# flydog-sdr/FlyDog_SDR_GPS

Measured on AMD Instinct MI355X. Metric: IQ Msamples/s ingested (waterfall + GPS acq); value = GPS acq, BASELINE configs[1], higher is better.
Workload: dtype f32

## Files before the change

### flydog_sdr_gps_amd/csrc/kg_acq.hip

```cpp
#include "kg_common.h"
#include "kg_fft.h"
#include "kg_acq_tables.h"

#include <math.h>
#include <stdlib.h>
#include <vector>

#define SUB      4096
#define NTAPS    31
#define DECIM    4


enum { SRC_BITS = 0, SRC_IQ16 = 1, SRC_CHIPS = 2 };

__constant__ float c_hb_even[16] = {
    -0.010233f,  0.010668f, -0.016324f,  0.024377f, -0.036482f,  0.056990f, -0.101993f,
     0.316926f,  0.316926f, -0.101993f,  0.056990f, -0.036482f,  0.024377f, -0.016324f,
     0.010668f, -0.010233f,
};
#define HB_CENTRE 0.500009f

KG_DEV float bipolar(int bit) { return bit ? -1.0f : 1.0f; }

template <int SRC>
KG_DEV cf acq_source(const void *__restrict__ src, int i, int nvalid, int nchips, int boc)
{
    if (i >= nvalid) return cf{0.f, 0.f};
    if constexpr (SRC == SRC_BITS) {
        const uint8_t *p = (const uint8_t *) src;
        const int bit = (p[i >> 3] >> (i & 7)) & 1;
        const int ph = i & 3;
        const int ls = ph < 2, lc = (ph == 0) | (ph == 3);
        return cf{bipolar(bit ^ ls), bipolar(bit ^ lc)};
    } else if constexpr (SRC == SRC_IQ16) {
        const short2 v = ((const short2 *) src)[i];
        const float a = (float) v.x, b = (float) v.y;
        switch (i & 3) {
        case 0:  return cf{a, b};
        case 1:  return cf{b, -a};
        case 2:  return cf{-a, -b};
        default: return cf{-b, a};
        }
    } else {
        const uint8_t *p = (const uint8_t *) src;
        const int chip = p[(i >> 4) % nchips];
        const int b11 = boc ? ((i & 15) >= 8) : 0;
        return cf{bipolar(chip ^ b11), 0.f};
    }
}

KG_DEV cf hb_tap(const float2 *x)
{
    cf acc = kg_scale(kg_ld(&x[0]), c_hb_even[0]);
#pragma unroll
    for (int j = 1; j < 16; j++) acc = acc + kg_scale(kg_ld(&x[2 * j]), c_hb_even[j]);
    acc = acc + kg_scale(kg_ld(&x[(NTAPS - 1) / 2]), HB_CENTRE);
    return acc;
}

#define FE_TILE 256
#define FE_NY1  (2 * FE_TILE + NTAPS - 2)
#define FE_NX   (2 * FE_NY1 + NTAPS - 2)

template <int SRC>
__global__ __launch_bounds__(256) void acq_frontend_kernel(const uint8_t *__restrict__ src,
                                                          size_t src_stride, int nvalid, int nchips, int boc,
                                                          float2 *__restrict__ td, int fft_len)
{
    __shared__ float2 xs[FE_NX + 1];
    __shared__ float2 y1[FE_NY1 + 1];
    const int tid = threadIdx.x;
    const int o0 = blockIdx.x * FE_TILE;
    const void *s = src + (size_t) blockIdx.y * src_stride;
    for (int u = tid; u < FE_NX; u += 256) kg_st(&xs[u], acq_source<SRC>(s, 4 * o0 + u, nvalid, nchips, boc));
    __syncthreads();
    for (int u = tid; u < FE_NY1; u += 256) kg_st(&y1[u], hb_tap(&xs[2 * u]));
    __syncthreads();
    kg_st(&td[(size_t) blockIdx.y * fft_len + o0 + tid], hb_tap(&y1[2 * tid]));
}

#define STAMP(i)                                                                      \
    do {                                                                              \
        if (STAMPS) {                                                                 \
            __builtin_amdgcn_sched_barrier(0);                                        \
            if (threadIdx.x == 0 && blockIdx.x == 0 && blockIdx.y == 0)               \
                stamps[i] = __builtin_amdgcn_s_memrealtime();                         \
            __builtin_amdgcn_sched_barrier(0);                                        \
        }                                                                             \
    } while (0)

template <bool STAMPS>
__global__ __launch_bounds__(256) void acq_fft_sub_kernel(const float2 *__restrict__ td,
                                                         float2 *__restrict__ scratch,
                                                         const float2 *__restrict__ tab4096, int P,
                                                         unsigned long long *__restrict__ stamps)
{
    extern __shared__ __attribute__((aligned(16))) float2 smem[];
    const int t = threadIdx.x, g = blockIdx.x;
    const float2 *in = td + (size_t) blockIdx.y * P * SUB;
    float2 *out = scratch + ((size_t) blockIdx.y * P + g) * SUB;
    STAMP(0);
    cf x[16], y[16];
#pragma unroll
    for (int j = 0; j < 16; j++) x[j] = kg_ld(&in[P * (t + 256 * j) + g]);
    kg_tw4096 tw;
    kg_tw4096_load(tw, tab4096, t);
    if (STAMPS) { asm volatile("s_waitcnt vmcnt(0)" ::: "memory"); }
    STAMP(1);
    kg_subfft4096<-1>(x, y, smem, smem + SUB, tw, t);
    STAMP(2);
#pragma unroll
    for (int m = 0; m < 16; m++) kg_st(&out[t + 256 * m], y[m]);
    if (STAMPS) { asm volatile("s_waitcnt vmcnt(0)" ::: "memory"); }
    STAMP(3);
}

template <int P>
__global__ __launch_bounds__(256) void acq_fft_combine_kernel(const float2 *__restrict__ scratch,
                                                             float2 *__restrict__ planes,
                                                             float2 *__restrict__ planes_b,
                                                             size_t planes_stride,
                                                             const float2 *__restrict__ tabN,
                                                             int halo)
{
    static_assert(P == 4 || P == 16, "N = 16384 or 65536");
    const int k = blockIdx.x * 256 + threadIdx.x;
    const float2 *f = scratch + (size_t) blockIdx.y * (P * SUB);
    cf v[P];
    v[0] = kg_ld(&f[k]);
#pragma unroll
    for (int g = 1; g < P; g++) v[g] = kg_cmulc(kg_ld(&f[g * SUB + k]), kg_ld(&tabN[g * k]));
    cf fq[P];
    if constexpr (P == 4) {
        kg_radix4<-1>(v[0], v[1], v[2], v[3]);
#pragma unroll
        for (int q = 0; q < 4; q++) fq[q] = v[q];
    } else {
        kg_radix16<-1>(v, fq);
    }
    if (planes) {
        const int row = 2 * (256 + 2 * halo), plane = 8 * row;
        float2 *o = planes + (size_t) blockIdx.y * planes_stride + (size_t) (k & (P - 1)) * plane;
#pragma unroll
        for (int q = 0; q < P; q++) {
            const int k1 = k / P + (SUB / P) * q;
            const int tt = k1 & 255, j = k1 >> 8;
            kg_st(&o[(j >> 1) * row + 2 * (tt + halo) + (j & 1)], fq[q]);
            if (tt < halo) {
                const int jj = (j - 1) & 15;
                kg_st(&o[(jj >> 1) * row + 2 * (tt + 256 + halo) + (jj & 1)], fq[q]);
            }
            if (tt >= 256 - halo) {
                const int jj = (j + 1) & 15;
                kg_st(&o[(jj >> 1) * row + 2 * (tt - 256 + halo) + (jj & 1)], fq[q]);
            }
        }
    }
    if (planes_b) {
        const int row = 2 * (512 + 2 * halo), plane = 4 * row;
        float2 *o = planes_b + (size_t) blockIdx.y * planes_stride + (size_t) (k & (P - 1)) * plane;
#pragma unroll
        for (int q = 0; q < P; q++) {
            const int k1 = k / P + (SUB / P) * q;
            const int ii = k1 & 511, j = k1 >> 9;
            kg_st(&o[(j >> 1) * row + 2 * (ii + halo) + (j & 1)], fq[q]);
            if (ii < halo) {
                const int jj = (j - 1) & 7;
                kg_st(&o[(jj >> 1) * row + 2 * (ii + 512 + halo) + (jj & 1)], fq[q]);
            }
            if (ii >= 512 - halo) {
                const int jj = (j + 1) & 7;
                kg_st(&o[(jj >> 1) * row + 2 * (ii - 512 + halo) + (jj & 1)], fq[q]);
            }
        }
    }
}

struct acq_red { float p; int i; float s; int pad; };

#define ACQ_CLAIM_STRIDE 32
#define ACQ_LDS_BYTES (2 * SUB * sizeof(float2) + 16)

struct __attribute__((aligned(16))) acq_part { float p; int i; float s; int pad; };

struct acq_pair_desc {
    int data_off;
    int code_off;
    int limit;
    int out;
};

struct acq_cell_desc { int data_off, code_off, dop, limit, out; };

struct acq_walk {
    int npairs;
    int ndop, dop_lo;
};

template <int P, bool STAMPS = false>
__global__ __launch_bounds__(256, 2) void acq_correlate_kernel(
    const float2 *__restrict__ data,
    const float2 *__restrict__ code,
    const float2 *__restrict__ tab4096, const float2 *__restrict__ tabN,
    const float2 *__restrict__ comb,
    const acq_pair_desc *__restrict__ pairs,
    int *__restrict__ claim,
    acq_walk walk,
    int halo,
    acq_part *__restrict__ parts,
    unsigned long long *__restrict__ stamps = nullptr)
{
    static_assert(P == 4 || P == 16, "N = 16384 or 65536");
    constexpr int LOGP = P == 4 ? 2 : 4;
    extern __shared__ __attribute__((aligned(16))) float2 smem[];
    float2 *tileA = smem, *tileB = smem + SUB;
    typedef __attribute__((address_space(3))) volatile int acq_lds_int;
    acq_lds_int *claim_slot = (acq_lds_int *) (smem + 2 * SUB);
    const int t = threadIdx.x;
    unsigned long long *st = (STAMPS && t == 0 && blockIdx.x == 8) ? stamps : nullptr;
    if (STAMPS && st) { st[0] = __builtin_amdgcn_s_memtime(); st[1] = __builtin_amdgcn_s_memrealtime(); }
    unsigned long long *wgt = (STAMPS && t == 0) ? stamps + 512 + 4 * blockIdx.x : nullptr;
    int wg_cells = 0;
    if (STAMPS && wgt) {
        wgt[0] = __builtin_amdgcn_s_memrealtime();
        wgt[2] = (unsigned long long) __builtin_amdgcn_s_getreg((20 << 0) | (0 << 6) | (31 << 11));
    }

    kg_tw4096 tw;
// ... 555 lines not shown
            const acq_part a1 = w[1], b1 = w[3];
            auto merge = [](acq_part &x, const acq_part &o) {
                const bool take = (o.p > x.p) | ((o.p == x.p) & (o.i < x.i));
                x.p = take ? o.p : x.p; x.i = take ? o.i : x.i;
                x.s += o.s;
            };
            merge(a, a1); merge(b, b1); merge(a, b);
            const float ave = a.s / (float) pd.limit;
            c.snr = a.p / ave;
            c.max_pwr = a.p; c.tot_pwr = a.s; c.idx = a.i;
            cells[(size_t) pd.out + di] = c;
        } else {
            c = cells[(size_t) pd.out + di];
        }
        if (c.snr > bs) { bs = c.snr; bd = di; bidx = c.idx; }
    }
#pragma unroll
    for (int off = 32; off >= 1; off >>= 1) {
        const float os = __shfl_xor(bs, off);
        const int od = __shfl_xor(bd, off), oi = __shfl_xor(bidx, off);
        if (os > bs || (os == bs && od < bd)) { bs = os; bd = od; bidx = oi; }
    }
    if (lane == 0) {
        kg_acq_result r;
        r.valid = bs > 0.f ? 1 : 0;
        r.snr = r.valid ? bs : 0.f;
        r.dop = r.valid ? dop_lo + bd : 0;
        r.idx = r.valid ? bidx : 0;
        out[p] = r;
    }
}

struct kg_acq {
    kg_ctx *ctx;
    int max_sats, dop_lo, dop_hi, ndop, max_blocks;
    int nsamples;
    int fft_len;
    int P;
    size_t in_stride;
    int halo;
    size_t code_len;
    const float2 *d_tabN;
    kg_dbuf<float2> own_tabN;
    kg_dbuf<float2> d_comb;
    kg_dbuf<float2> d_quart;
    kg_dbuf<float2> d_comb8;
    int grid8;
    kg_dbuf<float2> d_code;
    kg_dbuf<float2> d_data;
    kg_dbuf<float2> d_data_b;
    std::vector<char> code_layout;
    kg_dbuf<float2> d_td;
    kg_dbuf<float2> d_td_code;
    kg_dbuf<float2> d_fsub;
    kg_dbuf<float2> d_fsub_code;
    kg_dbuf<uint8_t> d_in;
    kg_hbuf<uint8_t> h_pin[4];
    hipEvent_t ev_pin[4];
    int pin_next;
    kg_hbuf<uint8_t> h_batch; size_t batch_cap; hipEvent_t ev_batch;
    hipStream_t cstream; hipEvent_t ev_in_free; bool in_free_set;
    kg_dbuf<uint8_t> d_chips;
    kg_dbuf<kg_acq_cell> d_cells;
    kg_dbuf<acq_part> d_parts;
    kg_dbuf<kg_acq_result> d_results;
    kg_dbuf<int> d_claim;
    std::vector<int> limits, code_set;
    std::vector<int> last_sats;
    const acq_pair_desc *d_pairs1, *d_pairs4;
    unsigned long pairs_seq;
    int last_first, last_nblocks, last_nsats, np1, np4, table_nblocks;
    hipStream_t fstream;
    bool own_fstream;
    std::vector<hipEvent_t> ev_ready, ev_done;
    std::vector<int> ready_of, done_of;
    int grid1;
};

static inline __host__ __device__ size_t plane_pos(int k1, int halo_col, int H, int layout)
{
    if (layout == 0) {
        const int t = k1 & 255, j = k1 >> 8, row = 2 * (256 + 2 * H);
        return (size_t) (j >> 1) * row + 2 * (t + halo_col + H) + (j & 1);
    }
    const int t = k1 & 511, j = k1 >> 9, row = 2 * (512 + 2 * H);
    return (size_t) (j >> 1) * row + 2 * (t + halo_col + H) + (j & 1);
}
static inline size_t spec_len(int P, int H) { return (size_t) P * 8 * 2 * (256 + 2 * H); }
static inline __host__ __device__ size_t plane_len(int H, int layout) { return layout == 0 ? (size_t) 8 * 2 * (256 + 2 * H) : (size_t) 4 * 2 * (512 + 2 * H); }

__global__ void acq_code_overrun_kernel(float2 *__restrict__ dst, int layout_dst, const float2 *__restrict__ src, int layout_src, int P, int H)
{
    const int t = blockIdx.x * blockDim.x + threadIdx.x;
    if (t >= P * H) return;
    const int k2 = t % P, k1 = t / P;
    const float2 v = src ? src[(size_t) k2 * plane_len(H, layout_src) + plane_pos(k1, 0, H, layout_src)] : make_float2(0.f, 0.f);
    const int T = layout_dst == 0 ? 256 : 512, J = SUB / T;
    dst[(size_t) k2 * plane_len(H, layout_dst) + plane_pos(k1 + T * (J - 1), T, H, layout_dst)] = v;
}

static void to_planes(const float *nat, std::vector<float2> &pl, int P, int H, int layout)
{
    const size_t plane = plane_len(H, layout);
    const int T = layout == 0 ? 256 : 512, J = SUB / T;
    pl.assign(spec_len(P, H), make_float2(0.f, 0.f));
    for (int k = 0; k < P * SUB; k++) {
        const float2 v = make_float2(nat[2 * k], nat[2 * k + 1]);
        const int k1 = k / P, t = k1 & (T - 1), j = k1 / T;
        float2 *p = pl.data() + (size_t) (k % P) * plane;
        p[plane_pos(k1, 0, H, layout)] = v;
        if (t < H) p[plane_pos(t + T * ((j - 1) & (J - 1)), T, H, layout)] = v;
        if (t >= T - H) p[plane_pos(t + T * ((j + 1) & (J - 1)), -T, H, layout)] = v;
    }
}
static void from_planes(const std::vector<float2> &pl, float *nat, int P, int H, int layout)
{
    const size_t plane = plane_len(H, layout);
    for (int k = 0; k < P * SUB; k++) {
        const float2 v = pl[(size_t) (k % P) * plane + plane_pos(k / P, 0, H, layout)];
        nat[2 * k] = v.x; nat[2 * k + 1] = v.y;
    }
}

static float2 unit_root(long k, long n)
{
    float2 r;
    kg_unit_root_f(k, n, &r.x, &r.y);
    return r;
}

template <int SRC>
static int launch_frontend(kg_acq *a, hipStream_t st, const uint8_t *d_src, size_t stride, int nbatch,
                           int nvalid, int nchips, int boc, float2 *d_td, float2 *d_scratch,
                           float2 *d_planes, float2 *d_planes_b, size_t planes_stride, int halo)
{
    kg_ctx *c = a->ctx;
    hipLaunchKernelGGL(acq_frontend_kernel<SRC>, dim3(a->fft_len / FE_TILE, nbatch), dim3(256), 0,
                       st, d_src, stride, nvalid, nchips, boc, d_td, a->fft_len);
    KG_HIP(hipGetLastError());
    hipLaunchKernelGGL(acq_fft_sub_kernel<false>, dim3(a->P, nbatch), dim3(256), 2 * SUB * sizeof(float2),
                       st, (const float2 *) d_td, d_scratch, (const float2 *) c->d_tab4096, a->P,
                       (unsigned long long *) nullptr);
    KG_HIP(hipGetLastError());
    if (a->P == 4)
        hipLaunchKernelGGL(acq_fft_combine_kernel<4>, dim3(SUB / 256, nbatch), dim3(256), 0, st,
                           (const float2 *) d_scratch, d_planes, d_planes_b, planes_stride,
                           (const float2 *) a->d_tabN, halo);
    else
        hipLaunchKernelGGL(acq_fft_combine_kernel<16>, dim3(SUB / 256, nbatch), dim3(256), 0, st,
                           (const float2 *) d_scratch, d_planes, d_planes_b, planes_stride,
                           (const float2 *) a->d_tabN, halo);
    KG_HIP(hipGetLastError());
    return KG_OK;
}

static int acq_init(kg_acq *a)
{
    kg_ctx *ctx = a->ctx;
    const int max_sats = a->max_sats, max_blocks = a->max_blocks, N = a->fft_len, P = a->P;
    {
        const int m = (a->dop_hi > -a->dop_lo ? a->dop_hi : -a->dop_lo);
        a->halo = (m + P - 1) / P + 2;
        a->code_len = spec_len(P, a->halo);
    }
    a->limits.assign(max_sats, 0); a->code_set.assign(max_sats, 0); a->code_layout.assign(max_sats, 0);
    a->last_first = a->last_nblocks = a->last_nsats = a->np1 = a->np4 = a->table_nblocks = 0;
    a->d_pairs1 = a->d_pairs4 = nullptr; a->pairs_seq = 0;
    a->in_stride = (size_t) a->nsamples * 4;
    const size_t spec = sizeof(float2) * N;
    if (N == 16384) a->d_tabN = ctx->d_tab16384;
    else {
        std::vector<float2> h(N);
        for (int k = 0; k < N; k++) h[k] = unit_root(k, N);
        KG_TRY(a->own_tabN.alloc(N, "kg_acq_create: twiddle table"));
        a->d_tabN = a->own_tabN;
        KG_HIP(hipMemcpy(a->own_tabN, h.data(), spec, hipMemcpyHostToDevice));
    }
    {
        std::vector<float2> comb(P * KG_ACQ_ROWK + (P == 16 ? 4 * 256 : 0)), quart(P * 4);
        static_assert(sizeof(float2) == 2 * sizeof(float), "float2 = (re, im)");
        kg_acq_row_consts(P, &comb[0].x);
        if (P == 16) kg_acq_mid_factors(N, &comb[P * KG_ACQ_ROWK].x);
        for (int k2 = 0; k2 < P; k2++)
            for (int q = 0; q < 4; q++) quart[4 * k2 + q] = unit_root((long) q * k2, P);
        KG_TRY(a->d_comb.alloc(comb.size(), "kg_acq_create: row constants"));
        KG_TRY(a->d_quart.alloc(quart.size(), "kg_acq_create: quarter factors"));
        KG_HIP(hipMemcpy(a->d_comb, comb.data(), sizeof(float2) * comb.size(), hipMemcpyHostToDevice));
        KG_HIP(hipMemcpy(a->d_quart, quart.data(), sizeof(float2) * quart.size(), hipMemcpyHostToDevice));
        std::vector<float2> comb8(P * 4);
        for (int k2 = 0; k2 < P; k2++)
            for (int k = 0; k < 4; k++) comb8[4 * k2 + k] = unit_root((long) (k + 1) * k2, N / 512);
        KG_TRY(a->d_comb8.alloc(comb8.size(), "kg_acq_create: combine constants"));
        KG_HIP(hipMemcpy(a->d_comb8, comb8.data(), sizeof(float2) * comb8.size(), hipMemcpyHostToDevice));
    }
    KG_TRY(a->d_code.alloc(a->code_len * max_sats, "kg_acq_create: code spectra"));
    KG_TRY(a->d_data.alloc((size_t) N * max_blocks, "kg_acq_create: data spectra"));
    KG_TRY(a->d_td.alloc((size_t) N * max_blocks, "kg_acq_create: decimated samples"));
    KG_TRY(a->d_td_code.alloc(N, "kg_acq_create: decimated samples"));
    KG_TRY(a->d_fsub.alloc((size_t) N * max_blocks, "kg_acq_create: sub-transforms"));
    KG_TRY(a->d_fsub_code.alloc(N, "kg_acq_create: sub-transforms"));
    KG_TRY(a->d_in.alloc(a->in_stride * max_blocks, "kg_acq_create: input staging"));
    for (int k = 0; k < 4; k++) {
        KG_TRY(a->h_pin[k].alloc(a->in_stride, "kg_acq_create: pinned input slots"));
        KG_HIP(hipEventCreateWithFlags(&a->ev_pin[k], hipEventDisableTiming));
    }
    KG_HIP(hipEventCreateWithFlags(&a->ev_batch, hipEventDisableTiming));
    KG_HIP(hipEventCreateWithFlags(&a->ev_in_free, hipEventDisableTiming));
    KG_TRY(kg_stream_get(ctx->device, &a->cstream));
    KG_TRY(a->d_chips.alloc(8192, "kg_acq_create: chips"));
    KG_TRY(a->d_cells.alloc((size_t) max_blocks * max_sats * a->ndop, "kg_acq_create: cells"));
    KG_TRY(a->d_parts.alloc(4 * (size_t) max_blocks * max_sats * a->ndop, "kg_acq_create: wave records"));
    KG_TRY(a->d_results.alloc((size_t) max_blocks * max_sats, "kg_acq_create: results"));
    KG_TRY(a->d_claim.alloc(16 * ACQ_CLAIM_STRIDE, "kg_acq_create: claim counters"));
    KG_HIP(hipMemset(a->d_claim, 0, sizeof(int) * 16 * ACQ_CLAIM_STRIDE));
    {
        const char *e = kg_tuning_env("KIWIGPU_ACQ_FRONT_STREAM");
        if (e && e[0] == '1') {
            KG_TRY(kg_stream_get(ctx->device, &a->fstream));
            a->own_fstream = true;
        }
    }
    a->ready_of.assign(max_blocks, -1); a->done_of.assign(max_blocks, -1);
    a->ev_ready.reserve(max_blocks); a->ev_done.reserve(max_blocks);
    for (int b = 0; b < max_blocks; b++) {
        hipEvent_t e1, e2;
        KG_HIP(hipEventCreateWithFlags(&e1, hipEventDisableTiming));
        a->ev_ready.push_back(e1);
        KG_HIP(hipEventCreateWithFlags(&e2, hipEventDisableTiming));
        a->ev_done.push_back(e2);
    }
    KG_HIP(hipMemset(a->d_data, 0, spec * max_blocks));
    KG_HIP(hipFuncSetAttribute((const void *) acq_fft_sub_kernel<false>,
                               hipFuncAttributeMaxDynamicSharedMemorySize, 2 * SUB * sizeof(float2)));
    KG_HIP(hipFuncSetAttribute((const void *) acq_fft_sub_kernel<true>,
                               hipFuncAttributeMaxDynamicSharedMemorySize, 2 * SUB * sizeof(float2)));
    int occ1 = 0;
#define ACQ_SETUP(PP)                                                                                          \
    KG_HIP(hipFuncSetAttribute((const void *) acq_correlate_kernel<PP>,                                       \
                               hipFuncAttributeMaxDynamicSharedMemorySize, ACQ_LDS_BYTES));                   \
    KG_HIP(hipOccupancyMaxActiveBlocksPerMultiprocessor(&occ1, acq_correlate_kernel<PP>, 256,                 \
                                                        ACQ_LDS_BYTES));
    if (P == 4) { ACQ_SETUP(4) } else { ACQ_SETUP(16) }
#undef ACQ_SETUP
    if (occ1 < 1) occ1 = 1;
    if (const char *e = kg_tuning_env("KIWIGPU_ACQ_WGS_PER_CU")) {
        const int v = atoi(e);
        if (v >= 1 && v < occ1) occ1 = v;
    }
    a->grid1 = (ctx->num_cus * occ1) & ~7;
    if (P == 4)
        KG_HIP(hipFuncSetAttribute((const void *) acq_correlate8_kernel<4>,
                                   hipFuncAttributeMaxDynamicSharedMemorySize, ACQ8_LDS_BYTES));
    else
        KG_HIP(hipFuncSetAttribute((const void *) acq_correlate8_kernel<16>,
                                   hipFuncAttributeMaxDynamicSharedMemorySize, ACQ8_LDS_BYTES));
    a->grid8 = ctx->num_cus & ~7;
    if (a->grid8 < 8) a->grid8 = 8;
    if (a->grid1 < 8) a->grid1 = 8;
    return KG_OK;
}

extern "C" {

int kg_acq_create_shape(kg_ctx *ctx, int max_sats, int dop_lo, int dop_hi, int max_blocks, int nsamples,
                        int fft_len, kg_acq **out)
{
    int rc = kg_ctx_use(ctx);
    if (rc) return rc;
    KG_REQUIRE(out != nullptr, KG_ERR_INVALID, "kg_acq_create: out is null");
    *out = nullptr;
    KG_REQUIRE(max_sats >= 1 && max_sats <= 4096, KG_ERR_INVALID, "kg_acq_create: max_sats %d", max_sats);
    KG_REQUIRE(dop_lo <= dop_hi && dop_lo >= -1000 && dop_hi <= 1000, KG_ERR_INVALID,
               "kg_acq_create: Doppler range %d..%d (supported: within -1000..1000)", dop_lo, dop_hi);
    KG_REQUIRE(max_blocks >= 1 && max_blocks <= 65535, KG_ERR_INVALID, "kg_acq_create: max_blocks %d",
               max_blocks);
    KG_REQUIRE(fft_len == 16384 || fft_len == 65536, KG_ERR_INVALID,
               "kg_acq_create: fft_len %d (supported: 16384, 65536)", fft_len);
    KG_REQUIRE(nsamples >= 8 && nsamples <= DECIM * fft_len && nsamples % 8 == 0, KG_ERR_INVALID,
               "kg_acq_create: nsamples %d (a multiple of 8, at most %d)", nsamples, DECIM * fft_len);
    KG_REQUIRE((size_t) max_blocks * fft_len < ((size_t) 1 << 31), KG_ERR_INVALID,
               "kg_acq_create: max_blocks %d x fft_len %d exceeds the 2^31-element offset range", max_blocks, fft_len);
    kg_acq *a = new (std::nothrow) kg_acq();
    KG_REQUIRE(a != nullptr, KG_ERR_NOMEM, "kg_acq_create: alloc");
    a->ctx = ctx; a->max_sats = max_sats; a->dop_lo = dop_lo; a->dop_hi = dop_hi;
    a->ndop = dop_hi - dop_lo + 1; a->max_blocks = max_blocks;
    a->nsamples = nsamples; a->fft_len = fft_len; a->P = fft_len / SUB;
    a->fstream = ctx->stream;
    rc = acq_init(a);
// ... 44 lines not shown
        from_planes(pl, nat.data(), a->P, 0, 0);
        to_planes(nat.data(), plb, a->P, 0, 1);
        memcpy(all.data() + (size_t) b * a->fft_len, plb.data(), sizeof(float2) * a->fft_len);
    }
    KG_REQUIRE(hipMemcpy(d, all.data(), sizeof(float2) * n, hipMemcpyHostToDevice) == hipSuccess, KG_ERR_HIP,
               "ensure_data_b: upload of layout B failed");
    a->d_data_b.p = d.p; d.p = nullptr;
    return KG_OK;
}

static int set_limit(kg_acq *a, int sat, int limit)
{
    KG_REQUIRE(sat >= 0 && sat < a->max_sats, KG_ERR_INVALID, "sat %d out of range (0..%d)", sat,
               a->max_sats - 1);
    KG_REQUIRE(limit >= 1 && limit <= 4 * SUB, KG_ERR_INVALID, "limit %d out of range (1..%d)", limit,
               4 * SUB);
    const int layout = limit > SUB ? 1 : 0;
    if (layout) {
        int rc = ensure_data_b(a);
        if (rc) return rc;
    }
    a->limits[sat] = limit;
    a->code_layout[sat] = layout;
    a->code_set[sat] = 1;
    a->last_sats.clear();
    return KG_OK;
}

static int acq_patch_overrun(kg_acq *a, int sat)
{
    if (sat < 0 || sat >= a->max_sats || !a->code_set[sat]) return KG_OK;
    const bool have_next = sat + 1 < a->max_sats && a->code_set[sat + 1];
    const int n = a->P * a->halo;
    hipLaunchKernelGGL(acq_code_overrun_kernel, dim3((n + 63) / 64), dim3(64), 0, a->ctx->stream,
                       a->d_code + (size_t) sat * a->code_len, a->code_layout[sat],
                       have_next ? (const float2 *) (a->d_code + (size_t) (sat + 1) * a->code_len) : (const float2 *) nullptr,
                       have_next ? a->code_layout[sat + 1] : 0, a->P, a->halo);
    KG_HIP(hipGetLastError());
    return KG_OK;
}

int kg_acq_set_code(kg_acq *a, int sat, const uint8_t *chips, int nchips, int boc, int limit)
{
    KG_REQUIRE(a && chips, KG_ERR_INVALID, "kg_acq_set_code: null argument");
    int rc = kg_ctx_use(a->ctx);
    if (rc) return rc;
    KG_REQUIRE(nchips >= 1 && nchips <= 8192, KG_ERR_INVALID, "kg_acq_set_code: nchips %d", nchips);
    for (int i = 0; i < nchips; i++)
        KG_REQUIRE(chips[i] <= 1, KG_ERR_INVALID, "kg_acq_set_code: chips[%d] = %d is not 0/1", i, chips[i]);
    KG_TRY(set_limit(a, sat, limit));
    KG_HIP(hipMemcpyAsync(a->d_chips, chips, nchips, hipMemcpyHostToDevice, a->ctx->stream));
    float2 *d_sv = a->d_code + (size_t) sat * a->code_len;
    rc = launch_frontend<SRC_CHIPS>(a, a->ctx->stream, a->d_chips, 0, 1, DECIM * a->fft_len, nchips, boc ? 1 : 0,
                                    a->d_td_code, a->d_fsub_code, a->code_layout[sat] ? nullptr : d_sv,
                                    a->code_layout[sat] ? d_sv : nullptr, a->code_len, a->halo);
    if (rc) return rc;
    if ((rc = acq_patch_overrun(a, sat)) || (rc = acq_patch_overrun(a, sat - 1))) return rc;
    KG_HIP(hipStreamSynchronize(a->ctx->stream));
    return KG_OK;
}

int kg_acq_set_code_fft(kg_acq *a, int sat, const float *code_fft, int limit)
{
    KG_REQUIRE(a && code_fft, KG_ERR_INVALID, "kg_acq_set_code_fft: null argument");
    int rc = kg_ctx_use(a->ctx);
    if (rc) return rc;
    KG_TRY(set_limit(a, sat, limit));
    std::vector<float2> pl;
    to_planes(code_fft, pl, a->P, a->halo, a->code_layout[sat]);
    KG_HIP(hipMemcpyAsync(a->d_code + (size_t) sat * a->code_len, pl.data(), sizeof(float2) * a->code_len,
                          hipMemcpyHostToDevice, a->ctx->stream));
    if ((rc = acq_patch_overrun(a, sat)) || (rc = acq_patch_overrun(a, sat - 1))) return rc;
    KG_HIP(hipStreamSynchronize(a->ctx->stream));
    return KG_OK;
}

static int get_planes(kg_acq *a, const float2 *d, float *nat, int H, int layout)
{
    std::vector<float2> pl(spec_len(a->P, H));
    KG_HIP(hipStreamSynchronize(a->fstream));
    KG_HIP(hipMemcpyAsync(pl.data(), d, sizeof(float2) * pl.size(), hipMemcpyDeviceToHost, a->ctx->stream));
    KG_HIP(hipStreamSynchronize(a->ctx->stream));
    from_planes(pl, nat, a->P, H, layout);
    return KG_OK;
}

int kg_acq_get_code_fft(kg_acq *a, int sat, float *code_fft)
{
    KG_REQUIRE(a && code_fft, KG_ERR_INVALID, "kg_acq_get_code_fft: null argument");
    int rc = kg_ctx_use(a->ctx);
    if (rc) return rc;
    KG_REQUIRE(sat >= 0 && sat < a->max_sats, KG_ERR_INVALID, "kg_acq_get_code_fft: sat %d", sat);
    KG_REQUIRE(a->code_set[sat], KG_ERR_STATE, "kg_acq_get_code_fft: no code set for sat %d", sat);
    return get_planes(a, a->d_code + (size_t) sat * a->code_len, code_fft, a->halo, a->code_layout[sat]);
}

static int check_block(kg_acq *a, int block, const void *p, const char *who)
{
    KG_REQUIRE(a && p, KG_ERR_INVALID, "%s: null argument", who);
    KG_REQUIRE(block >= 0 && block < a->max_blocks, KG_ERR_INVALID, "%s: block %d out of range (0..%d)",
               who, block, a->max_blocks - 1);
    return kg_ctx_use(a->ctx);
}

__global__ __launch_bounds__(256) void acq_stage_copy_kernel(const uint4 *__restrict__ src, uint4 *__restrict__ dst, size_t n16)
{
    const size_t i = (size_t) blockIdx.x * 256 + threadIdx.x;
// ... 7 lines not shown
    KG_HIP(hipEventSynchronize(a->ev_pin[k]));
    memcpy(a->h_pin[k], src, bytes);
    if ((bytes & 15) == 0 && bytes >= 65536) {
        const size_t n16 = bytes / 16;
        hipLaunchKernelGGL(acq_stage_copy_kernel, dim3((unsigned) ((n16 + 255) / 256)), dim3(256), 0, a->fstream,
                           (const uint4 *) a->h_pin[k].p, (uint4 *) d_stage, n16);
        KG_HIP(hipGetLastError());
    } else {
        KG_HIP(hipMemcpyAsync(d_stage, a->h_pin[k], bytes, hipMemcpyHostToDevice, a->fstream));
    }
    KG_HIP(hipEventRecord(a->ev_pin[k], a->fstream));
    return KG_OK;
}
static int staging_consumed(kg_acq *a)
{
    KG_HIP(hipEventRecord(a->ev_in_free, a->fstream));
    a->in_free_set = true;
    return KG_OK;
}

static int wait_once(hipStream_t st, const std::vector<hipEvent_t> &ev, const std::vector<int> &of, int b, int n)
{
    for (int i = b; i < b + n; i++) {
        const int e = of[i];
        if (e < 0) continue;
        bool seen = false;
        for (int k = b; k < i && !seen; k++) seen = of[k] == e;
        if (!seen) KG_HIP(hipStreamWaitEvent(st, ev[e], 0));
    }
    return KG_OK;
}
static int front_begin(kg_acq *a, int b, int n = 1)
{
    if (!a->own_fstream) return KG_OK;
    return wait_once(a->fstream, a->ev_done, a->done_of, b, n);
}
static int front_end(kg_acq *a, int b, int n = 1)
{
    if (!a->own_fstream) return KG_OK;
    KG_HIP(hipEventRecord(a->ev_ready[b], a->fstream));
    for (int i = b; i < b + n; i++) a->ready_of[i] = b;
    return KG_OK;
}

}

template <int SRC>
static int sample_dev(kg_acq *a, int first, int nblocks, const void *d_src, size_t stride)
{
    int rc;
    KG_TRY(front_begin(a, first, nblocks));
    const size_t off = (size_t) first * a->fft_len;
    rc = launch_frontend<SRC>(a, a->fstream, (const uint8_t *) d_src, stride, nblocks, a->nsamples, 0, 0,
                              a->d_td + off, a->d_fsub + off, a->d_data + off, a->d_data_b ? a->d_data_b + off : nullptr,
                              a->fft_len, 0);
    if (rc) return rc;
    return front_end(a, first, nblocks);
}

extern "C" {

int kg_acq_sample_bits_dev(kg_acq *a, int block, const void *d_packed)
{
    int rc = check_block(a, block, d_packed, "kg_acq_sample_bits_dev");
    if (rc) return rc;
    return sample_dev<SRC_BITS>(a, block, 1, d_packed, 0);
}

int kg_acq_sample_bits(kg_acq *a, int block, const uint8_t *packed)
{
    int rc = check_block(a, block, packed, "kg_acq_sample_bits");
    if (rc) return rc;
    uint8_t *stage = a->d_in + a->in_stride * block;
    if ((rc = stage_host_block(a, stage, packed, (size_t) a->nsamples / 8))) return rc;
    KG_TRY(sample_dev<SRC_BITS>(a, block, 1, stage, 0));
    return staging_consumed(a);
}

int kg_acq_sample_iq16_dev(kg_acq *a, int block, const void *d_iq)
{
    int rc = check_block(a, block, d_iq, "kg_acq_sample_iq16_dev");
    if (rc) return rc;
    KG_REQUIRE(((uintptr_t) d_iq & 3) == 0, KG_ERR_INVALID, "kg_acq_sample_iq16_dev: pointer not 4-byte aligned");
    return sample_dev<SRC_IQ16>(a, block, 1, d_iq, 0);
}

int kg_acq_sample_iq16_batch_dev(kg_acq *a, int first, int nblocks, const void *d_iq, size_t stride_bytes)
{
    int rc = check_block(a, first, d_iq, "kg_acq_sample_iq16_batch_dev");
    if (rc) return rc;
    KG_REQUIRE(nblocks >= 1 && first + nblocks <= a->max_blocks, KG_ERR_INVALID,
               "kg_acq_sample_iq16_batch_dev: blocks %d..%d (max %d)", first, first + nblocks - 1, a->max_blocks);
    KG_REQUIRE(((uintptr_t) d_iq & 3) == 0 && (stride_bytes & 3) == 0, KG_ERR_INVALID,
               "kg_acq_sample_iq16_batch_dev: pointer/stride not 4-byte aligned");
    return sample_dev<SRC_IQ16>(a, first, nblocks, d_iq, stride_bytes);
}

int kg_acq_sample_iq16_batch(kg_acq *a, int first, int nblocks, const int16_t *iq, size_t stride_samples)
{
    int rc = check_block(a, first, iq, "kg_acq_sample_iq16_batch");
    if (rc) return rc;
    KG_REQUIRE(nblocks >= 1 && first + nblocks <= a->max_blocks, KG_ERR_INVALID,
               "kg_acq_sample_iq16_batch: blocks %d..%d (max %d)", first, first + nblocks - 1, a->max_blocks);
    KG_REQUIRE(stride_samples >= (size_t) a->nsamples, KG_ERR_INVALID, "kg_acq_sample_iq16_batch: stride %zu < %d samples",
               stride_samples, a->nsamples);
    const size_t bytes = a->in_stride * (size_t) nblocks;
    KG_HIP(hipEventSynchronize(a->ev_batch));
// ... 203 lines not shown
        if (a->P == 4) {
            KG_HIP(hipFuncSetAttribute((const void *) acq_correlate8_kernel<4, true>,
                                       hipFuncAttributeMaxDynamicSharedMemorySize, ACQ8_LDS_BYTES));
            hipLaunchKernelGGL((acq_correlate8_kernel<4, true>), dim3(a->grid8), dim3(512), ACQ8_LDS_BYTES, st,
                               (const float2 *) a->d_data_b, (const float2 *) a->d_code, (const float2 *) a->ctx->d_tab4096,
                               (const float2 *) a->d_tabN, (const float2 *) a->d_comb8, (const float2 *) a->d_quart,
                               a->d_pairs4, a->d_claim + 8 * ACQ_CLAIM_STRIDE, w, a->halo, a->d_cells, d);
        } else {
            KG_HIP(hipFuncSetAttribute((const void *) acq_correlate8_kernel<16, true>,
                                       hipFuncAttributeMaxDynamicSharedMemorySize, ACQ8_LDS_BYTES));
            hipLaunchKernelGGL((acq_correlate8_kernel<16, true>), dim3(a->grid8), dim3(512), ACQ8_LDS_BYTES, st,
                               (const float2 *) a->d_data_b, (const float2 *) a->d_code, (const float2 *) a->ctx->d_tab4096,
                               (const float2 *) a->d_tabN, (const float2 *) a->d_comb8, (const float2 *) a->d_quart,
                               a->d_pairs4, a->d_claim + 8 * ACQ_CLAIM_STRIDE, w, a->halo, a->d_cells, d);
        }
        KG_HIP(hipGetLastError());
        KG_HIP(hipMemsetAsync(a->d_claim, 0, sizeof(int) * 16 * ACQ_CLAIM_STRIDE, st));
        KG_HIP(hipStreamSynchronize(st));
        KG_HIP(hipMemcpy(stamps, d, bytes, hipMemcpyDeviceToHost));
        return KG_OK;
    }
    KG_REQUIRE(a->np1 > 0, KG_ERR_STATE, "kg_acq_debug_corr_stamps: no C/A SV in the list");
    unsigned long long *d = nullptr;
    const size_t bytes = sizeof(unsigned long long) * (512 + 4 * 1024);
    KG_REQUIRE(a->grid1 <= 1024, KG_ERR_STATE, "kg_acq_debug_corr_stamps: grid %d", a->grid1);
    kg_scope tmp(a->ctx);
    KG_TRY(tmp.alloc(&d, 512 + 4 * 1024, "kg_acq_debug_corr_stamps"));
    KG_HIP(hipMemset(d, 0, bytes));
    KG_HIP(hipMemsetAsync(a->d_claim, 0, sizeof(int) * 16 * ACQ_CLAIM_STRIDE, st));
    if (a->P == 4) {
        KG_HIP(hipFuncSetAttribute((const void *) acq_correlate_kernel<4, true>,
                                   hipFuncAttributeMaxDynamicSharedMemorySize, ACQ_LDS_BYTES));
        launch_correlate<4, true>(a, st, 0, a->d_pairs1, a->np1, d);
    } else {
        KG_HIP(hipFuncSetAttribute((const void *) acq_correlate_kernel<16, true>,
                                   hipFuncAttributeMaxDynamicSharedMemorySize, ACQ_LDS_BYTES));
        launch_correlate<16, true>(a, st, 0, a->d_pairs1, a->np1, d);
    }
    KG_HIP(hipGetLastError());
    KG_HIP(hipMemsetAsync(a->d_claim, 0, sizeof(int) * 16 * ACQ_CLAIM_STRIDE, st));
    KG_HIP(hipStreamSynchronize(st));
    KG_HIP(hipMemcpy(stamps, d, bytes, hipMemcpyDeviceToHost));
    return KG_OK;
}

int kg_acq_debug_fft_stamps(kg_acq *a, int block, unsigned long long *stamps, int n)
{
    int rc = check_block(a, block, stamps, "kg_acq_debug_fft_stamps");
    if (rc) return rc;
    KG_REQUIRE(n >= 4, KG_ERR_INVALID, "kg_acq_debug_fft_stamps: need room for 4 stamps");
    kg_ctx *c = a->ctx;
    unsigned long long *d = nullptr;
    kg_scope tmp(c);
    KG_TRY(tmp.alloc(&d, 8, "kg_acq_debug_fft_stamps"));
    KG_HIP(hipStreamSynchronize(a->fstream));
    for (int rep = 0; rep < 3; rep++) {
        hipLaunchKernelGGL(acq_fft_sub_kernel<true>, dim3(a->P, 1), dim3(256), 2 * SUB * sizeof(float2),
                           c->stream, (const float2 *) (a->d_td + (size_t) block * a->fft_len),
                           a->d_fsub + (size_t) block * a->fft_len, (const float2 *) c->d_tab4096, a->P, d);
        KG_HIP(hipGetLastError());
        KG_HIP(hipStreamSynchronize(c->stream));
    }
    KG_HIP(hipMemcpy(stamps, d, 4 * sizeof(unsigned long long), hipMemcpyDeviceToHost));
    return KG_OK;
}

}
```

Baseline: 2674.

## Fuse FFT sub-transforms and combine into one decimation-in-frequency forward kernel

Replaces the two-pass FFT (4096-point sub-FFTs on strided inputs written to scratch, then a radix-4/16 combine kernel scattering into correlation planes) with one kernel. Each block first does the radix-P butterfly plus twiddle on contiguous loads, then a 4096-point FFT, and writes plane rows directly with vectorized stores. This removes the scratch buffer round trip and one launch. It also restructures the half-band decimation front end into polyphase even/odd LDS layouts with per-thread register taps and vector output stores. The cost is more register pressure and redundant global reads in the P=16 path, since each block reloads all 16 segments.

```diff
diff --git a/flydog_sdr_gps_amd/csrc/kg_acq.hip b/flydog_sdr_gps_amd/csrc/kg_acq.hip
--- a/flydog_sdr_gps_amd/csrc/kg_acq.hip
+++ b/flydog_sdr_gps_amd/csrc/kg_acq.hip
@@ -49,34 +49,62 @@
     }
 }
 
-KG_DEV cf hb_tap(const float2 *x)
-{
-    cf acc = kg_scale(kg_ld(&x[0]), c_hb_even[0]);
-#pragma unroll
-    for (int j = 1; j < 16; j++) acc = acc + kg_scale(kg_ld(&x[2 * j]), c_hb_even[j]);
-    acc = acc + kg_scale(kg_ld(&x[(NTAPS - 1) / 2]), HB_CENTRE);
-    return acc;
+template <int K>
+KG_DEV void hb_taps(const cf (&e)[K + 15], const cf (&o)[K], cf (&y)[K])
+{
+#pragma unroll
+    for (int k = 0; k < K; k++) {
+        cf acc = kg_scale(e[k], c_hb_even[0]);
+#pragma unroll
+        for (int j = 1; j < 16; j++) acc = acc + kg_scale(e[k + j], c_hb_even[j]);
+        y[k] = acc + kg_scale(o[k], HB_CENTRE);
+    }
 }
 
 #define FE_TILE 256
 #define FE_NY1  (2 * FE_TILE + NTAPS - 2)
 #define FE_NX   (2 * FE_NY1 + NTAPS - 2)
+#define FE_XS 168
+#define FE_YS 144
 
 template <int SRC>
 __global__ __launch_bounds__(256) void acq_frontend_kernel(const uint8_t *__restrict__ src,
                                                           size_t src_stride, int nvalid, int nchips, int boc,
                                                           float2 *__restrict__ td, int fft_len)
 {
-    __shared__ float2 xs[FE_NX + 1];
-    __shared__ float2 y1[FE_NY1 + 1];
+    __shared__ float2 xe[4 * FE_XS], xo[4 * FE_XS];
+    __shared__ __attribute__((aligned(16))) float2 ye[2 * FE_YS], yo[2 * FE_YS];
     const int tid = threadIdx.x;
     const int o0 = blockIdx.x * FE_TILE;
     const void *s = src + (size_t) blockIdx.y * src_stride;
-    for (int u = tid; u < FE_NX; u += 256) kg_st(&xs[u], acq_source<SRC>(s, 4 * o0 + u, nvalid, nchips, boc));
+    for (int u = tid; u < FE_NX; u += 256) {
+        const int i = u >> 1;
+        kg_st(&((u & 1) ? xo : xe)[(i & 3) * FE_XS + (i >> 2)], acq_source<SRC>(s, 4 * o0 + u, nvalid, nchips, boc));
+    }
     __syncthreads();
-    for (int u = tid; u < FE_NY1; u += 256) kg_st(&y1[u], hb_tap(&xs[2 * u]));
+    if (tid < (FE_NY1 + 3) / 4) {
+        cf e[19], o[4], y[4];
+#pragma unroll
+        for (int m = 0; m < 19; m++) e[m] = kg_ld(&xe[(m & 3) * FE_XS + tid + (m >> 2)]);
+#pragma unroll
+        for (int k = 0; k < 4; k++) o[k] = kg_ld(&xo[((7 + k) & 3) * FE_XS + tid + ((7 + k) >> 2)]);
+        hb_taps<4>(e, o, y);
+        kg_st(&ye[tid], y[0]);
+        if (4 * tid + 1 < FE_NY1) kg_st(&yo[tid], y[1]);
+        if (4 * tid + 2 < FE_NY1) kg_st(&ye[FE_YS + tid], y[2]);
+        if (4 * tid + 3 < FE_NY1) kg_st(&yo[FE_YS + tid], y[3]);
+    }
     __syncthreads();
-    kg_st(&td[(size_t) blockIdx.y * fft_len + o0 + tid], hb_tap(&y1[2 * tid]));
+    if (tid < FE_TILE / 2) {
+        cf e[17], o[2], y[2];
+#pragma unroll
+        for (int m = 0; m < 17; m++) e[m] = kg_ld(&ye[(m & 1) * FE_YS + tid + (m >> 1)]);
+#pragma unroll
+        for (int k = 0; k < 2; k++) o[k] = kg_ld(&yo[((7 + k) & 1) * FE_YS + tid + ((7 + k) >> 1)]);
+        hb_taps<2>(e, o, y);
+        typedef float cf2 __attribute__((ext_vector_type(4)));
+        *reinterpret_cast<cf2 *>(&td[(size_t) blockIdx.y * fft_len + o0 + 2 * tid]) = cf2{y[0].x, y[0].y, y[1].x, y[1].y};
+    }
 }
 
 #define STAMP(i)                                                                      \
@@ -89,91 +117,121 @@
         }                                                                             \
     } while (0)
 
-template <bool STAMPS>
-__global__ __launch_bounds__(256) void acq_fft_sub_kernel(const float2 *__restrict__ td,
-                                                         float2 *__restrict__ scratch,
-                                                         const float2 *__restrict__ tab4096, int P,
-                                                         unsigned long long *__restrict__ stamps)
-{
+KG_DEV cf acq_radix4_out(cf x0, cf x1, cf x2, cf x3, int r)
+{
+    if (r & 1) {
+        const cf d02 = x0 - x2, d13 = x1 - x3;
+        return (r & 2) ? kg_addj(d02, d13) : kg_subj(d02, d13);
+    }
+    const cf s02 = x0 + x2, s13 = x1 + x3;
+    return (r & 2) ? s02 - s13 : s02 + s13;
+}
+
+KG_DEV void acq_store_plane(const cf (&y)[16], float2 *__restrict__ pa, float2 *__restrict__ pb, int t, int halo)
+{
+    typedef float cf2 __attribute__((ext_vector_type(4)));
+    if (pa) {
+        const int row = 2 * (256 + 2 * halo);
+#pragma unroll
+        for (int i = 0; i < 8; i++)
+            *reinterpret_cast<cf2 *>(&pa[i * row + 2 * (t + halo)]) = cf2{y[2 * i].x, y[2 * i].y, y[2 * i + 1].x, y[2 * i + 1].y};
+        if (t < halo) {
+#pragma unroll
+            for (int j = 0; j < 16; j++) {
+                const int jj = (j - 1) & 15;
+                kg_st(&pa[(jj >> 1) * row + 2 * (t + 256 + halo) + (jj & 1)], y[j]);
+            }
+        }
+        if (t >= 256 - halo) {
+#pragma unroll
+            for (int j = 0; j < 16; j++) {
+                const int jj = (j + 1) & 15;
+                kg_st(&pa[(jj >> 1) * row + 2 * (t - 256 + halo) + (jj & 1)], y[j]);
+            }
+        }
+    }
+    if (pb) {
+        const int row = 2 * (512 + 2 * halo);
+#pragma unroll
+        for (int i = 0; i < 8; i++) {
+            const int m = 4 * (i >> 1) + (i & 1);
+            *reinterpret_cast<cf2 *>(&pb[(i >> 1) * row + 2 * (t + 256 * (i & 1) + halo)]) =
+                cf2{y[m].x, y[m].y, y[m + 2].x, y[m + 2].y};
+        }
+        if (t < halo) {
+#pragma unroll
+            for (int j = 0; j < 8; j++) {
+                const int jj = (j - 1) & 7;
+                kg_st(&pb[(jj >> 1) * row + 2 * (t + 512 + halo) + (jj & 1)], y[2 * j]);
+            }
+        }
+        if (t >= 256 - halo) {
+#pragma unroll
+            for (int j = 0; j < 8; j++) {
+                const int jj = (j + 1) & 7;
+                kg_st(&pb[(jj >> 1) * row + 2 * (t - 256 + halo) + (jj & 1)], y[2 * j + 1]);
+            }
+        }
+    }
+}
+
+template <int P, bool STAMPS>
+__global__ __launch_bounds__(256) void acq_fft_forward_kernel(const float2 *__restrict__ td,
+                                                             float2 *__restrict__ planes,
+                                                             float2 *__restrict__ planes_b,
+                                                             size_t planes_stride,
+                                                             const float2 *__restrict__ tab4096,
+                                                             const float2 *__restrict__ tabN,
+                                                             int halo,
+                                                             unsigned long long *__restrict__ stamps)
+{
+    static_assert(P == 4 || P == 16, "N = 16384 or 65536");
     extern __shared__ __attribute__((aligned(16))) float2 smem[];
-    const int t = threadIdx.x, g = blockIdx.x;
-    const float2 *in = td + (size_t) blockIdx.y * P * SUB;
-    float2 *out = scratch + ((size_t) blockIdx.y * P + g) * SUB;
+    const int t = threadIdx.x, r = blockIdx.x;
+    const float2 *in = td + (size_t) blockIdx.y * (P * SUB);
     STAMP(0);
     cf x[16], y[16];
-#pragma unroll
-    for (int j = 0; j < 16; j++) x[j] = kg_ld(&in[P * (t + 256 * j) + g]);
+    if constexpr (P == 4) {
+        cf a[4][16];
+#pragma unroll
+        for (int q = 0; q < 4; q++)
+#pragma unroll
+            for (int j = 0; j < 16; j++) a[q][j] = kg_ld(&in[SUB * q + t + 256 * j]);
+#pragma unroll
+        for (int j = 0; j < 16; j++) x[j] = acq_radix4_out(a[0][j], a[1][j], a[2][j], a[3][j], r);
+    } else {
+        const cf w1 = kg_ld(&tabN[(r & 15) * (SUB * P / 16)]), w2 = kg_ld(&tabN[((2 * r) & 15) * (SUB * P / 16)]),
+                 w3 = kg_ld(&tabN[((3 * r) & 15) * (SUB * P / 16)]);
+#pragma unroll
+        for (int j = 0; j < 16; j++) {
+            cf a[16];
+#pragma unroll
+            for (int q = 0; q < 16; q++) a[q] = kg_ld(&in[SUB * q + t + 256 * j]);
+            cf u[4];
+#pragma unroll
+            for (int b = 0; b < 4; b++) u[b] = acq_radix4_out(a[b], a[4 + b], a[8 + b], a[12 + b], r & 3);
+            kg_cmul3v<true>(u[1], u[2], u[3], w1, w2, w3);
+            x[j] = (u[0] + u[2]) + (u[1] + u[3]);
+        }
+    }
+    if (r) {
+        cf w[16];
+#pragma unroll
+        for (int j = 0; j < 16; j++) w[j] = kg_ld(&tabN[r * (t + 256 * j)]);
+#pragma unroll
+        for (int j = 0; j < 16; j += 4) kg_cmul4v<true>(x[j], x[j + 1], x[j + 2], x[j + 3], w[j], w[j + 1], w[j + 2], w[j + 3]);
+    }
     kg_tw4096 tw;
     kg_tw4096_load(tw, tab4096, t);
     if (STAMPS) { asm volatile("s_waitcnt vmcnt(0)" ::: "memory"); }
     STAMP(1);
     kg_subfft4096<-1>(x, y, smem, smem + SUB, tw, t);
     STAMP(2);
-#pragma unroll
-    for (int m = 0; m < 16; m++) kg_st(&out[t + 256 * m], y[m]);
+    const size_t spec = (size_t) blockIdx.y * planes_stride;
+    acq_store_plane(y, planes ? planes + spec + (size_t) r * (8 * 2 * (256 + 2 * halo)) : nullptr,
+                    planes_b ? planes_b + spec + (size_t) r * (4 * 2 * (512 + 2 * halo)) : nullptr, t, halo);
     if (STAMPS) { asm volatile("s_waitcnt vmcnt(0)" ::: "memory"); }
     STAMP(3);
-}
-
-template <int P>
-__global__ __launch_bounds__(256) void acq_fft_combine_kernel(const float2 *__restrict__ scratch,
-                                                             float2 *__restrict__ planes,
-                                                             float2 *__restrict__ planes_b,
-                                                             size_t planes_stride,
-                                                             const float2 *__restrict__ tabN,
-                                                             int halo)
-{
-    static_assert(P == 4 || P == 16, "N = 16384 or 65536");
-    const int k = blockIdx.x * 256 + threadIdx.x;
-    const float2 *f = scratch + (size_t) blockIdx.y * (P * SUB);
-    cf v[P];
-    v[0] = kg_ld(&f[k]);
-#pragma unroll
-    for (int g = 1; g < P; g++) v[g] = kg_cmulc(kg_ld(&f[g * SUB + k]), kg_ld(&tabN[g * k]));
-    cf fq[P];
-    if constexpr (P == 4) {
-        kg_radix4<-1>(v[0], v[1], v[2], v[3]);
-#pragma unroll
-        for (int q = 0; q < 4; q++) fq[q] = v[q];
-    } else {
-        kg_radix16<-1>(v, fq);
-    }
-    if (planes) {
-        const int row = 2 * (256 + 2 * halo), plane = 8 * row;
-        float2 *o = planes + (size_t) blockIdx.y * planes_stride + (size_t) (k & (P - 1)) * plane;
-#pragma unroll
-        for (int q = 0; q < P; q++) {
-            const int k1 = k / P + (SUB / P) * q;
-            const int tt = k1 & 255, j = k1 >> 8;
-            kg_st(&o[(j >> 1) * row + 2 * (tt + halo) + (j & 1)], fq[q]);
-            if (tt < halo) {
-                const int jj = (j - 1) & 15;
-                kg_st(&o[(jj >> 1) * row + 2 * (tt + 256 + halo) + (jj & 1)], fq[q]);
-            }
-            if (tt >= 256 - halo) {
-                const int jj = (j + 1) & 15;
-                kg_st(&o[(jj >> 1) * row + 2 * (tt - 256 + halo) + (jj & 1)], fq[q]);
-            }
-        }
-    }
-    if (planes_b) {
-        const int row = 2 * (512 + 2 * halo), plane = 4 * row;
-        float2 *o = planes_b + (size_t) blockIdx.y * planes_stride + (size_t) (k & (P - 1)) * plane;
-#pragma unroll
-        for (int q = 0; q < P; q++) {
-            const int k1 = k / P + (SUB / P) * q;
-            const int ii = k1 & 511, j = k1 >> 9;
-            kg_st(&o[(j >> 1) * row + 2 * (ii + halo) + (j & 1)], fq[q]);
-            if (ii < halo) {
-                const int jj = (j - 1) & 7;
-                kg_st(&o[(jj >> 1) * row + 2 * (ii + 512 + halo) + (jj & 1)], fq[q]);
-            }
-            if (ii >= 512 - halo) {
-                const int jj = (j + 1) & 7;
-                kg_st(&o[(jj >> 1) * row + 2 * (ii - 512 + halo) + (jj & 1)], fq[q]);
-            }
-        }
-    }
 }
 
 struct acq_red { float p; int i; float s; int pad; };
@@ -835,8 +893,6 @@
     std::vector<char> code_layout;
     kg_dbuf<float2> d_td;
     kg_dbuf<float2> d_td_code;
-    kg_dbuf<float2> d_fsub;
-    kg_dbuf<float2> d_fsub_code;
     kg_dbuf<uint8_t> d_in;
     kg_hbuf<uint8_t> h_pin[4];
     hipEvent_t ev_pin[4];
@@ -914,25 +970,21 @@
 
 template <int SRC>
 static int launch_frontend(kg_acq *a, hipStream_t st, const uint8_t *d_src, size_t stride, int nbatch,
-                           int nvalid, int nchips, int boc, float2 *d_td, float2 *d_scratch,
+                           int nvalid, int nchips, int boc, float2 *d_td,
                            float2 *d_planes, float2 *d_planes_b, size_t planes_stride, int halo)
 {
     kg_ctx *c = a->ctx;
     hipLaunchKernelGGL(acq_frontend_kernel<SRC>, dim3(a->fft_len / FE_TILE, nbatch), dim3(256), 0,
                        st, d_src, stride, nvalid, nchips, boc, d_td, a->fft_len);
     KG_HIP(hipGetLastError());
-    hipLaunchKernelGGL(acq_fft_sub_kernel<false>, dim3(a->P, nbatch), dim3(256), 2 * SUB * sizeof(float2),
-                       st, (const float2 *) d_td, d_scratch, (const float2 *) c->d_tab4096, a->P,
-                       (unsigned long long *) nullptr);
-    KG_HIP(hipGetLastError());
     if (a->P == 4)
-        hipLaunchKernelGGL(acq_fft_combine_kernel<4>, dim3(SUB / 256, nbatch), dim3(256), 0, st,
-                           (const float2 *) d_scratch, d_planes, d_planes_b, planes_stride,
-                           (const float2 *) a->d_tabN, halo);
+        hipLaunchKernelGGL((acq_fft_forward_kernel<4, false>), dim3(4, nbatch), dim3(256), 2 * SUB * sizeof(float2), st,
+                           (const float2 *) d_td, d_planes, d_planes_b, planes_stride, (const float2 *) c->d_tab4096,
+                           (const float2 *) a->d_tabN, halo, (unsigned long long *) nullptr);
     else
-        hipLaunchKernelGGL(acq_fft_combine_kernel<16>, dim3(SUB / 256, nbatch), dim3(256), 0, st,
-                           (const float2 *) d_scratch, d_planes, d_planes_b, planes_stride,
-                           (const float2 *) a->d_tabN, halo);
+        hipLaunchKernelGGL((acq_fft_forward_kernel<16, false>), dim3(16, nbatch), dim3(256), 2 * SUB * sizeof(float2), st,
+                           (const float2 *) d_td, d_planes, d_planes_b, planes_stride, (const float2 *) c->d_tab4096,
+                           (const float2 *) a->d_tabN, halo, (unsigned long long *) nullptr);
     KG_HIP(hipGetLastError());
     return KG_OK;
 }
@@ -980,8 +1032,6 @@
     KG_TRY(a->d_data.alloc((size_t) N * max_blocks, "kg_acq_create: data spectra"));
     KG_TRY(a->d_td.alloc((size_t) N * max_blocks, "kg_acq_create: decimated samples"));
     KG_TRY(a->d_td_code.alloc(N, "kg_acq_create: decimated samples"));
-    KG_TRY(a->d_fsub.alloc((size_t) N * max_blocks, "kg_acq_create: sub-transforms"));
-    KG_TRY(a->d_fsub_code.alloc(N, "kg_acq_create: sub-transforms"));
     KG_TRY(a->d_in.alloc(a->in_stride * max_blocks, "kg_acq_create: input staging"));
     for (int k = 0; k < 4; k++) {
         KG_TRY(a->h_pin[k].alloc(a->in_stride, "kg_acq_create: pinned input slots"));
@@ -1013,10 +1063,12 @@
         a->ev_done.push_back(e2);
     }
     KG_HIP(hipMemset(a->d_data, 0, spec * max_blocks));
-    KG_HIP(hipFuncSetAttribute((const void *) acq_fft_sub_kernel<false>,
-                               hipFuncAttributeMaxDynamicSharedMemorySize, 2 * SUB * sizeof(float2)));
-    KG_HIP(hipFuncSetAttribute((const void *) acq_fft_sub_kernel<true>,
-                               hipFuncAttributeMaxDynamicSharedMemorySize, 2 * SUB * sizeof(float2)));
+    if (P == 4)
+        KG_HIP(hipFuncSetAttribute((const void *) acq_fft_forward_kernel<4, false>,
+                                   hipFuncAttributeMaxDynamicSharedMemorySize, 2 * SUB * sizeof(float2)));
+    else
+        KG_HIP(hipFuncSetAttribute((const void *) acq_fft_forward_kernel<16, false>,
+                                   hipFuncAttributeMaxDynamicSharedMemorySize, 2 * SUB * sizeof(float2)));
     int occ1 = 0;
 #define ACQ_SETUP(PP)                                                                                          \
     KG_HIP(hipFuncSetAttribute((const void *) acq_correlate_kernel<PP>,                                       \
@@ -1167,7 +1219,7 @@
     KG_HIP(hipMemcpyAsync(a->d_chips, chips, nchips, hipMemcpyHostToDevice, a->ctx->stream));
     float2 *d_sv = a->d_code + (size_t) sat * a->code_len;
     rc = launch_frontend<SRC_CHIPS>(a, a->ctx->stream, a->d_chips, 0, 1, DECIM * a->fft_len, nchips, boc ? 1 : 0,
-                                    a->d_td_code, a->d_fsub_code, a->code_layout[sat] ? nullptr : d_sv,
+                                    a->d_td_code, a->code_layout[sat] ? nullptr : d_sv,
                                     a->code_layout[sat] ? d_sv : nullptr, a->code_len, a->halo);
     if (rc) return rc;
     if ((rc = acq_patch_overrun(a, sat)) || (rc = acq_patch_overrun(a, sat - 1))) return rc;
@@ -1281,7 +1333,7 @@
     KG_TRY(front_begin(a, first, nblocks));
     const size_t off = (size_t) first * a->fft_len;
     rc = launch_frontend<SRC>(a, a->fstream, (const uint8_t *) d_src, stride, nblocks, a->nsamples, 0, 0,
-                              a->d_td + off, a->d_fsub + off, a->d_data + off, a->d_data_b ? a->d_data_b + off : nullptr,
+                              a->d_td + off, a->d_data + off, a->d_data_b ? a->d_data_b + off : nullptr,
                               a->fft_len, 0);
     if (rc) return rc;
     return front_end(a, first, nblocks);
@@ -1591,12 +1643,25 @@
     kg_ctx *c = a->ctx;
     unsigned long long *d = nullptr;
     kg_scope tmp(c);
+    float2 *d_planes = nullptr;
     KG_TRY(tmp.alloc(&d, 8, "kg_acq_debug_fft_stamps"));
+    KG_TRY(tmp.alloc(&d_planes, a->fft_len, "kg_acq_debug_fft_stamps"));
     KG_HIP(hipStreamSynchronize(a->fstream));
+    const float2 *d_td = a->d_td + (size_t) block * a->fft_len;
     for (int rep = 0; rep < 3; rep++) {
-        hipLaunchKernelGGL(acq_fft_sub_kernel<true>, dim3(a->P, 1), dim3(256), 2 * SUB * sizeof(float2),
-                           c->stream, (const float2 *) (a->d_td + (size_t) block * a->fft_len),
-                           a->d_fsub + (size_t) block * a->fft_len, (const float2 *) c->d_tab4096, a->P, d);
+        if (a->P == 4) {
+            KG_HIP(hipFuncSetAttribute((const void *) acq_fft_forward_kernel<4, true>,
+                                       hipFuncAttributeMaxDynamicSharedMemorySize, 2 * SUB * sizeof(float2)));
+            hipLaunchKernelGGL((acq_fft_forward_kernel<4, true>), dim3(4, 1), dim3(256), 2 * SUB * sizeof(float2), c->stream,
+                               d_td, d_planes, (float2 *) nullptr, (size_t) a->fft_len, (const float2 *) c->d_tab4096,
+                               (const float2 *) a->d_tabN, 0, d);
+        } else {
+            KG_HIP(hipFuncSetAttribute((const void *) acq_fft_forward_kernel<16, true>,
+                                       hipFuncAttributeMaxDynamicSharedMemorySize, 2 * SUB * sizeof(float2)));
+            hipLaunchKernelGGL((acq_fft_forward_kernel<16, true>), dim3(16, 1), dim3(256), 2 * SUB * sizeof(float2), c->stream,
+                               d_td, d_planes, (float2 *) nullptr, (size_t) a->fft_len, (const float2 *) c->d_tab4096,
+                               (const float2 *) a->d_tabN, 0, d);
+        }
         KG_HIP(hipGetLastError());
         KG_HIP(hipStreamSynchronize(c->stream));
     }
```

Result: no change. 2678, median of 6 (+0.1%).
